# deepinv/deepinv

Hardware: NVIDIA H100
Metric: pnp_pgd_iterations_per_s (higher is better)
Workload: dtype f32 (3 x FP16 split-operand tensor-core GEMMs: 22-bit operands, fp32 accumulate) + f32 operators

## Files before the change

deepinv_b200/csrc/conv_tc32.cu:

```cuda
#include "common.cuh"
#ifndef DINVK_EMUL
#include "tc_ptx.cuh"
#include "tma_tile.cuh"
#include <cuda_fp16.h>
#else
namespace dinvk { namespace tc {
inline void ldg256(const void* p, uint32_t (&r)[8]) { std::memcpy(r, p, 32); }
inline void stg256(void* p, const uint32_t (&r)[8]) { std::memcpy(p, r, 32); }
} }
#endif

#include <algorithm>
#include <cstdlib>
#include <cstring>

namespace dinvk {
namespace t32 {

constexpr int TX = 16, TY = 8;
constexpr int A_TILE = 128 * 128;
constexpr int B_TILE = 128 * 128;
constexpr int STAGE = 2 * A_TILE + B_TILE;
constexpr int STAGES = 4;
constexpr int SMEM = STAGES * STAGE + 1024;
constexpr int THREADS = 2 * 128 + 32;

__device__ __forceinline__ float rna_tf32(float x) {
#ifndef DINVK_EMUL
  uint32_t u;
  asm("cvt.rna.tf32.f32 %0, %1;" : "=r"(u) : "f"(x));
  return __uint_as_float(u);
#else
  return __uint_as_float((__float_as_uint(x) + 0x1000u) & 0xffffe000u);
#endif
}

struct FmtTF32 {
  using elem = float;
  static constexpr int CH = 16, EB = 4, ID = 0;
  static constexpr float CORR = 1.0f;
#ifndef DINVK_EMUL
  static constexpr CUtensorMapDataType TM = CU_TENSOR_MAP_DATA_TYPE_FLOAT32;
#endif
};
struct FmtF16 {
  using elem = __half;
  static constexpr int CH = 32, EB = 2, ID = 1;
  static constexpr float CORR = 4.8828125e-4f;
#ifndef DINVK_EMUL
  static constexpr CUtensorMapDataType TM = CU_TENSOR_MAP_DATA_TYPE_FLOAT16;
#endif
};

#ifndef DINVK_EMUL
template <class F, int N>
__device__ __forceinline__ void mma(float* d, uint32_t a_lo, uint32_t a_hi, uint32_t b_lo, uint32_t b_hi, uint32_t accumulate) {
  if constexpr (F::ID == 0) {
    if constexpr (N == 128) tc::wgmma_tf32_n128(d, a_lo, a_hi, b_lo, b_hi, accumulate);
    else tc::wgmma_tf32_n64(d, a_lo, a_hi, b_lo, b_hi, accumulate);
  } else {
    if constexpr (N == 128) tc::wgmma_f16_n128(d, a_lo, a_hi, b_lo, b_hi, accumulate);
    else tc::wgmma_f16_n64(d, a_lo, a_hi, b_lo, b_hi, accumulate);
  }
}
template <class F>
__device__ __forceinline__ void mma_block(float* acc, uint32_t a, uint32_t a_hi, uint32_t b, uint32_t b_hi, uint32_t fresh) {
  mma<F, 128>(acc, a, a_hi, b, b_hi, fresh);
  mma<F, 128>(acc, a + 2, a_hi, b + 2, b_hi, 1u);
  mma<F, 64>(acc + 32, a + 4, a_hi, b, b_hi, 1u);
  mma<F, 64>(acc + 32, a + 6, a_hi, b + 2, b_hi, 1u);
}
template <class F>
__device__ __forceinline__ void mma_block64(float* acc, uint32_t a, uint32_t a_hi, uint32_t b, uint32_t b_hi, uint32_t fresh) {
  mma<F, 64>(acc, a, a_hi, b, b_hi, fresh);
  mma<F, 64>(acc + 32, a, a_hi, b + 512, b_hi, fresh);
  mma<F, 64>(acc, a + 2, a_hi, b + 2, b_hi, 1u);
  mma<F, 64>(acc + 32, a + 2, a_hi, b + 514, b_hi, 1u);
  mma<F, 64>(acc + 32, a + 4, a_hi, b, b_hi, 1u);
  mma<F, 64>(acc + 32, a + 6, a_hi, b + 2, b_hi, 1u);
}
template <class F>
__device__ __forceinline__ void drain(float* v, const float* acc) {
#pragma unroll
  for (int i = 0; i < 32; ++i) v[i] += acc[i] + acc[32 + i] * F::CORR;
}

__device__ __forceinline__ void release_stage(uint64_t* bar) {
  __syncwarp();
  if ((threadIdx.x & 31) == 0) tc::mbar_arrive(bar);
}

struct Maps {
  CUtensorMap a[4];
  CUtensorMap b;
};

struct Params {
  int B, H, W, Cin, Cout;
  int ntaps, kc_per_tap;
  int dx[9], dy[9], amap[9];
  int mode;
  int tiles_x, tiles_y, n_tiles;
  int relu;
  int win;
  const void* res;
  const void* res2;
  void* out;
  int* flag;
  const float* bias;
  int ngrp;
};

// ... 32 lines not shown
  return bad;
}
template <class F>
__device__ __forceinline__ void add_split_raw(const uint32_t (*raw)[8], float* v) {
  if constexpr (F::ID == 0) {
#pragma unroll
    for (int e = 0; e < 8; ++e) {
      v[e] += __uint_as_float(raw[0][e]) + __uint_as_float(raw[2][e]);
      v[8 + e] += __uint_as_float(raw[1][e]) + __uint_as_float(raw[3][e]);
    }
  } else {
#pragma unroll
    for (int c = 0; c < 2; ++c)
#pragma unroll
      for (int e = 0; e < 8; ++e) {
        const float2 h = __half22float2(*reinterpret_cast<const __half2*>(&raw[c][e]));
        const float2 l = __half22float2(*reinterpret_cast<const __half2*>(&raw[2 + c][e]));
        v[c * 16 + 2 * e] += h.x + l.x * F::CORR;
        v[c * 16 + 2 * e + 1] += h.y + l.y * F::CORR;
      }
  }
}
template <class F>
__device__ __forceinline__ void add_split(const typename F::elem* p, float* v) {
  uint32_t raw[4][8];
  const char* pc = reinterpret_cast<const char*>(p);
#pragma unroll
  for (int k = 0; k < 4; ++k) tc::ldg256(pc + 32 * k, raw[k]);
  add_split_raw<F>(raw, v);
}

#ifndef DINVK_EMUL
template <class F>
__device__ __forceinline__ void add_split_pair(const typename F::elem* p, float& a, float& b) {
  if constexpr (F::ID == 0) {
    const float2 h = __ldg(reinterpret_cast<const float2*>(p)), l = __ldg(reinterpret_cast<const float2*>(p + F::CH));
    a += h.x + l.x;
    b += h.y + l.y;
  } else {
    const float2 h = __half22float2(__ldg(reinterpret_cast<const __half2*>(p)));
    const float2 l = __half22float2(__ldg(reinterpret_cast<const __half2*>(p + F::CH)));
    a += h.x + l.x * F::CORR;
    b += h.y + l.y * F::CORR;
  }
}
template <class F>
__device__ __forceinline__ bool store_split_pair(typename F::elem* p, float a, float b) {
  if constexpr (F::ID == 0) {
    const float ha = rna_tf32(a), hb = rna_tf32(b);
    *reinterpret_cast<float2*>(p) = make_float2(ha, hb);
    *reinterpret_cast<float2*>(p + F::CH) = make_float2(a - ha, b - hb);
    return false;
  } else {
    const __half h0 = __float2half_rn(a), h1 = __float2half_rn(b);
    const __half l0 = __float2half_rn((a - __half2float(h0)) * 2048.0f), l1 = __float2half_rn((b - __half2float(h1)) * 2048.0f);
    *reinterpret_cast<__half2*>(p) = __halves2half2(h0, h1);
    *reinterpret_cast<__half2*>(p + F::CH) = __halves2half2(l0, l1);
    return !(fabsf(a) < 65000.0f) || !(fabsf(b) < 65000.0f);
  }
}

template <class F>
__device__ __forceinline__ void epilogue_split(const Params& P, float* v, int b, const int (&y)[2], const int (&x)[2], int n0) {
  using E = typename F::elem;
  const int q = threadIdx.x & 3;
  const int tap = P.mode == 2 ? n0 / P.Cout : 0;
  const int c0 = n0 - tap * P.Cout;
  bool bad = false;
#pragma unroll
  for (int r = 0; r < 2; ++r) {
    if (!(y[r] < P.H && x[r] < P.W)) continue;
    long long pix;
    if (P.mode == 2) pix = ((long long)b * (2 * P.H) + 2 * y[r] + (tap >> 1)) * (2LL * P.W) + 2 * x[r] + (tap & 1);
    else pix = ((long long)b * P.H + y[r]) * P.W + x[r];
#pragma unroll
    for (int j = 0; j < 8; ++j) {
      const int c = c0 + 8 * j + 2 * q;
      float a = v[4 * j + 2 * r], bb = v[4 * j + 2 * r + 1];
      if (P.bias) { a += __ldg(P.bias + c); bb += __ldg(P.bias + c + 1); }
      if (P.relu) { a = fmaxf(a, 0.f); bb = fmaxf(bb, 0.f); }
      const long long o = pix * P.Cout * 2 + (c / F::CH) * 2 * F::CH + (c % F::CH);
      if (P.res) add_split_pair<F>(static_cast<const E*>(P.res) + o, a, bb);
      if (P.res2) add_split_pair<F>(static_cast<const E*>(P.res2) + o, a, bb);
      bad |= store_split_pair<F>(static_cast<E*>(P.out) + o, a, bb);
    }
  }
  if (bad && P.flag) atomicOr(P.flag, 1);
}

template <class F>
__global__ void __launch_bounds__(THREADS, 1) conv_tc32_kernel(const __grid_constant__ Maps M, const Params P) {
  extern __shared__ uint8_t smem_raw[];
  uint8_t* smem = reinterpret_cast<uint8_t*>((reinterpret_cast<uintptr_t>(smem_raw) + 1023) & ~static_cast<uintptr_t>(1023));
  __shared__ __align__(8) uint64_t full_bar[STAGES];
  __shared__ __align__(8) uint64_t empty_bar[STAGES];

  const int warp = threadIdx.x >> 5, lane = threadIdx.x & 31;
  const int pixel_tiles = P.B * P.tiles_y * P.tiles_x;
  const int total_tiles = pixel_tiles * P.n_tiles;
  const int nk = P.ntaps * P.kc_per_tap;

  if (threadIdx.x == 0) {
    tc::prefetch_tmap(&M.a[0]);
    tc::prefetch_tmap(&M.b);
    for (int s = 0; s < STAGES; ++s) { tc::mbar_init(&full_bar[s], 1); tc::mbar_init(&empty_bar[s], 8); }
    tc::fence_barrier_init();
  }
  __syncthreads();

  if (warp == 8) {
    if (lane == 0) {
      int s = 0; uint32_t ph = 0;
      for (int t = blockIdx.x; t < total_tiles; t += gridDim.x) {
        int pt, nt; tile_index(P, pixel_tiles, t, pt, nt);
        const int b = pt / (P.tiles_y * P.tiles_x), r = pt - b * (P.tiles_y * P.tiles_x);
        const int y0 = (r / P.tiles_x) * TY, x0 = (r % P.tiles_x) * TX;
        for (int kb = 0; kb < nk; ++kb) {
          const int tap = kb / P.kc_per_tap, kc = kb - tap * P.kc_per_tap;
          tc::mbar_wait(&empty_bar[s], ph ^ 1);
          uint8_t* sa = smem + s * STAGE;
          tc::mbar_arrive_expect_tx(&full_bar[s], STAGE);
          tc::tma_load_4d(sa, &M.a[P.amap[tap]], &full_bar[s], (2 * kc) * (2 * F::CH), x0 + P.dx[tap], y0 + P.dy[tap], b);
          tc::tma_load_4d(sa + A_TILE, &M.a[P.amap[tap]], &full_bar[s], (2 * kc + 1) * (2 * F::CH), x0 + P.dx[tap], y0 + P.dy[tap], b);
          tc::tma_load_2d(sa + 2 * A_TILE, &M.b, &full_bar[s], tap * P.Cin + kc * (2 * F::CH), nt * 128);
          if (++s == STAGES) { s = 0; ph ^= 1; }
        }
      }
    }
  } else {
    const int wg = warp >> 2;
    constexpr uint32_t HI = tc::desc_hi_sw128(1024);
    const uint32_t smem_lo = tc::smem_u32(smem) >> 4;
    float acc[64], v[32];
#pragma unroll
    for (int i = 0; i < 64; ++i) acc[i] = 0.f;
    int s = 0; uint32_t ph = 0;
    for (int t = blockIdx.x; t < total_tiles; t += gridDim.x) {
      int pt, nt; tile_index(P, pixel_tiles, t, pt, nt);
      const int b = pt / (P.tiles_y * P.tiles_x), r = pt - b * (P.tiles_y * P.tiles_x);
      const int y0 = (r / P.tiles_x) * TY, x0 = (r % P.tiles_x) * TX;
#pragma unroll
      for (int i = 0; i < 32; ++i) v[i] = 0.f;
      int in_win = 0, pend = -1;
      for (int kb = 0; kb < nk; ++kb) {
        tc::mbar_wait(&full_bar[s], ph);
        const uint32_t a0 = smem_lo + static_cast<uint32_t>(s) * (STAGE >> 4) + static_cast<uint32_t>(wg * (64 * 128 >> 4));
        const uint32_t b0 = smem_lo + static_cast<uint32_t>(s) * (STAGE >> 4) + (2 * A_TILE >> 4);
        tc::wgmma_fence();
#pragma unroll
        for (int jj = 0; jj < 2; ++jj)
          mma_block<F>(acc, a0 + jj * (A_TILE >> 4), HI, b0 + jj * 4, HI, (jj | in_win) != 0 ? 1u : 0u);
        tc::wgmma_commit();
        if (++in_win == P.win || kb == nk - 1) {
          tc::wgmma_wait<0>();
          tc::reg_fence<64>(acc);
          if (pend >= 0) release_stage(&empty_bar[pend]);
          release_stage(&empty_bar[s]);
          pend = -1;
          drain<F>(v, acc);
          in_win = 0;
        } else {
          tc::wgmma_wait<1>();
          if (pend >= 0) release_stage(&empty_bar[pend]);
          pend = s;
        }
        if (++s == STAGES) { s = 0; ph ^= 1; }
      }
      int y[2], x[2];
#pragma unroll
      for (int rr = 0; rr < 2; ++rr) {
        const int m = 64 * wg + 16 * (warp & 3) + (lane >> 2) + 8 * rr;
        y[rr] = y0 + m / TX; x[rr] = x0 + m % TX;
      }
      epilogue_split<F>(P, v, b, y, x, nt * 64);
    }
  }
}

namespace slab {
constexpr int TXP = 16, TYP = 16;
constexpr int SLAB_X = TXP + 8, SLAB_Y = TYP + 2;
constexpr int SLAB_BYTES = SLAB_X * SLAB_Y * 128;
constexpr int A_STAGES = 2, B_STAGES = 6;
constexpr int WT_TILE = 128 * 128;
constexpr int SMEM_BYTES = A_STAGES * SLAB_BYTES + B_STAGES * WT_TILE + 1024;
constexpr int CONSUMER_WARPS = 8;
constexpr int THREADS = 32 * CONSUMER_WARPS + 128;
constexpr int PRODUCER_REGS = 40, CONSUMER_REGS = 232;
static_assert(SLAB_BYTES % 1024 == 0, "slab stages must stay 1024-byte aligned");
static_assert(SMEM_BYTES <= 227 * 1024, "shared memory budget");
}

template <class F>
__global__ void __launch_bounds__(slab::THREADS, 1) conv_tc32_slab_kernel(const __grid_constant__ Maps M, const Params P) {
  using namespace slab;
  extern __shared__ uint8_t smem_raw[];
  uint8_t* smem = reinterpret_cast<uint8_t*>((reinterpret_cast<uintptr_t>(smem_raw) + 1023) & ~static_cast<uintptr_t>(1023));
  uint8_t* smem_b = smem + A_STAGES * SLAB_BYTES;
  __shared__ __align__(8) uint64_t afull[A_STAGES];
  __shared__ __align__(8) uint64_t aempty[A_STAGES];
  __shared__ __align__(8) uint64_t bfull[B_STAGES];
  __shared__ __align__(8) uint64_t bempty[B_STAGES];

  const int warp = threadIdx.x >> 5, lane = threadIdx.x & 31;
  const int pixel_tiles = P.B * P.tiles_y * P.tiles_x;
  const int total_tiles = pixel_tiles * P.n_tiles;
  const int nblk = P.Cin / F::CH;

  if (threadIdx.x == 0) {
    tc::prefetch_tmap(&M.a[0]);
    tc::prefetch_tmap(&M.b);
    for (int s = 0; s < A_STAGES; ++s) { tc::mbar_init(&afull[s], 1); tc::mbar_init(&aempty[s], CONSUMER_WARPS); }
    for (int s = 0; s < B_STAGES; ++s) { tc::mbar_init(&bfull[s], 1); tc::mbar_init(&bempty[s], CONSUMER_WARPS); }
    tc::fence_barrier_init();
  }
  __syncthreads();

  if (warp >= CONSUMER_WARPS) {
    tc::setmaxnreg_dec<PRODUCER_REGS>();
// ... 51 lines not shown
          tc::wgmma_fence();
#pragma unroll
          for (int par = 0; par < 2; ++par) {
            const int tap = 2 * tp + par;
            if (tap < 9) {
              const uint32_t a_t = slab_lo + static_cast<uint32_t>((tap / 3) * SLAB_X + (tap % 3)) * 8;
              mma_block64<F>(acc0, a_t, HI_A, b_lo + par * 4, HI_B, tap == 0 ? fresh : 1u);
              mma_block64<F>(acc1, a_t + BLK1, HI_A, b_lo + par * 4, HI_B, tap == 0 ? fresh : 1u);
            }
          }
          tc::wgmma_commit();
          if (tp == 4) {
            tc::wgmma_wait<0>();
            tc::reg_fence<64>(acc0);
            tc::reg_fence<64>(acc1);
            if (pend_b >= 0) release_stage(&bempty[pend_b]);
            release_stage(&bempty[sb]);
            release_stage(&aempty[sa]);
            pend_b = -1;
            if (last_of_win) {
              drain<F>(v0, acc0);
              drain<F>(v1, acc1);
            }
          } else {
            tc::wgmma_wait<1>();
            if (pend_b >= 0) release_stage(&bempty[pend_b]);
            pend_b = sb;
          }
          if (++sb == B_STAGES) { sb = 0; phb ^= 1; }
        }
        if (++sa == A_STAGES) { sa = 0; pha ^= 1; }
        in_win = last_of_win ? 0 : in_win + 1;
      }
      int y[2], x[2];
#pragma unroll
      for (int rr = 0; rr < 2; ++rr) {
        const int m = 16 * (warp & 3) + (lane >> 2) + 8 * rr;
        y[rr] = y0 + 8 * wg + (m >> 3); x[rr] = x0 + (m & 7);
      }
      epilogue_split<F>(P, v0, b, y, x, nt * 64);
#pragma unroll
      for (int rr = 0; rr < 2; ++rr) x[rr] += 8;
      epilogue_split<F>(P, v1, b, y, x, nt * 64);
    }
  }
}

#endif
struct HeadParams {
  const float* x; const float* w; const float* bias; void* out;
  int B, C, H, W, Cout;
  float fill_scalar; const float* fill_batch; int has_fill; int relu;
  int* flag;
};

template <class F, int CT>
__global__ void __launch_bounds__(256) head_tc32_kernel(const HeadParams P) {
  constexpr int KR = 9 * CT, KP = (KR + 3) & ~3;
#ifndef DINVK_EMUL
  extern __shared__ __align__(16) float sw[];
#else
  float* sw = reinterpret_cast<float*>(::emul::dyn_smem());
#endif
  for (int i = threadIdx.x; i < P.Cout * KP; i += blockDim.x) {
    const int co = i / KP, k = i - co * KP;
    sw[i] = k < KR ? __ldg(P.w + co * KR + k) : 0.f;
  }
  __syncthreads();
  const long long npix = (long long)P.B * P.H * P.W;
  const long long p = (long long)blockIdx.x * blockDim.x + threadIdx.x;
  if (p >= npix) return;
  const long long HW = (long long)P.H * P.W;
  const int b = (int)(p / HW);
  const int rem = (int)(p - (long long)b * HW);
  const int y = rem / P.W, x = rem - y * P.W;
  const float fillv = P.has_fill ? (P.fill_batch ? __ldg(P.fill_batch + b) : P.fill_scalar) : 0.f;
// ... 363 lines not shown
    out[(b * C + c) * HW + hw] = (float)s[0] + (float)s[F::CH] * F::CORR;
  }
}
template <class F>
__global__ void __launch_bounds__(256) nchw_to_split_kernel(const float* __restrict__ in, typename F::elem* __restrict__ out, int C, int H, int W,
                                                            long long n) {
  const long long stride = (long long)gridDim.x * blockDim.x;
  const long long HW = (long long)H * W;
  for (long long i = (long long)blockIdx.x * blockDim.x + threadIdx.x; i < n; i += stride) {
    const long long pix = i / C;
    const int c = (int)(i - pix * C);
    const long long b = pix / HW, hw = pix - b * HW;
    const float v = __ldg(in + (b * C + c) * HW + hw);
    typename F::elem* d = out + pix * C * 2 + (c / F::CH) * 2 * F::CH + (c % F::CH);
    if constexpr (F::ID == 0) {
      const float hi = rna_tf32(v);
      d[0] = hi;
      d[F::CH] = v - hi;
    } else {
      const __half hi = __float2half_rn(v);
      d[0] = hi;
      d[F::CH] = __float2half_rn((v - __half2float(hi)) * 2048.0f);
    }
  }
}

#ifndef DINVK_EMUL
template <class F>
static int map_split(CUtensorMap* m, const void* ptr, int rank, const uint64_t* dims, const uint64_t* strides, const uint32_t* box,
                     const char* what) {
  return encode_tiled(m, F::TM, rank, ptr, dims, strides, box, CU_TENSOR_MAP_SWIZZLE_128B, CU_TENSOR_MAP_L2_PROMOTION_L2_256B, what);
}

static int default_window() {
  static int w = -1;
  if (w < 0) {
    const char* e = getenv("DINVK_TC32_WINDOW");
    w = e ? std::max(1, atoi(e)) : 4;
  }
  return w;
}

template <class F>
static int conv_generic(const void* x, const void* weight, const float* bias, const void* res, const void* res2, void* out, int B, int H,
                        int W, int Cin, int Cout, int kind, int act, int window, int* flag, void* stream) {
  DINVK_CHECK_ARG(x && weight && out, "conv_tc32: null pointer");
  DINVK_CHECK_ARG(B >= 0 && H >= 1 && W >= 1, "conv_tc32: bad shape");
  DINVK_CHECK_ARG(kind >= 0 && kind <= 2, "conv_tc32: kind=%d not in 0..2", kind);
  DINVK_CHECK_ARG(Cin % (2 * F::CH) == 0 && Cin >= 2 * F::CH, "conv_tc32: Cin=%d must be a multiple of %d", Cin, 2 * F::CH);
  DINVK_CHECK_ARG(Cout % 64 == 0 && Cout >= 64, "conv_tc32: Cout=%d must be a multiple of 64", Cout);
  DINVK_CHECK_ARG(kind != 1 || (H % 2 == 0 && W % 2 == 0), "conv_tc32: 2x2 stride-2 needs even H, W");
  DINVK_CHECK_ARG(kind == 0 || (!res && !res2), "conv_tc32: residual inputs are for kind 0 only");
  if (B == 0) return DINVK_OK;
  Maps M;
  Params P{};
  int rc;
  const uint64_t px = (uint64_t)Cin * 2 * F::EB;
  P.B = B; P.Cin = Cin; P.Cout = Cout;
  P.kc_per_tap = Cin / (2 * F::CH);
  P.relu = act; P.res = res; P.res2 = res2; P.out = out; P.bias = bias; P.flag = flag;
  P.win = window > 0 ? window : default_window();
  const uint32_t abox[4] = {2 * F::CH, TX, TY, 1};
  long long K = Cin, rows = 2LL * Cout;
  if (kind == 1) {
    const int Ho = H / 2, Wo = W / 2;
    const uint64_t adims[4] = {(uint64_t)Cin * 2, (uint64_t)Wo, (uint64_t)Ho, (uint64_t)B}, astrides[3] = {2 * px, 2 * px * W, px * W * H};
    for (int t = 0; t < 4; ++t) {
      const char* base = reinterpret_cast<const char*>(x) + ((long long)(t >> 1) * W + (t & 1)) * px;
      if ((rc = map_split<F>(&M.a[t], base, 4, adims, astrides, abox, "tc32 activations"))) return rc;
      P.amap[t] = t;
    }
    K = 4LL * Cin;
    P.H = Ho; P.W = Wo; P.ntaps = 4; P.n_tiles = Cout / 64;
  } else {
    const uint64_t adims[4] = {(uint64_t)Cin * 2, (uint64_t)W, (uint64_t)H, (uint64_t)B}, astrides[3] = {px, px * W, px * W * H};
    if ((rc = map_split<F>(&M.a[0], x, 4, adims, astrides, abox, "tc32 activations"))) return rc;
    M.a[1] = M.a[0]; M.a[2] = M.a[0]; M.a[3] = M.a[0];
    P.H = H; P.W = W;
    if (kind == 0) {
      K = 9LL * Cin;
      P.ntaps = 9; P.n_tiles = Cout / 64;
      for (int t = 0; t < 9; ++t) { P.dx[t] = t % 3 - 1; P.dy[t] = t / 3 - 1; }
    } else {
      rows = 8LL * Cout;
      P.ntaps = 1; P.mode = 2; P.n_tiles = 4 * Cout / 64;
    }
  }
  const uint64_t wdims[2] = {(uint64_t)K, (uint64_t)rows}, wstride = (uint64_t)K * F::EB;
  const uint32_t wbox[2] = {2 * F::CH, 128};
  if ((rc = map_split<F>(&M.b, weight, 2, wdims, &wstride, wbox, "tc32 weights"))) return rc;
  P.tiles_x = ceil_div(P.W, TX); P.tiles_y = ceil_div(P.H, TY);
  P.ngrp = getenv("DINVK_TC32_NT_OUTER") ? 1 : P.n_tiles;
  return launch_persistent(conv_tc32_kernel<F>, THREADS, SMEM, (long long)P.B * P.tiles_y * P.tiles_x * P.n_tiles, stream, M, P);
}

template <class F>
static int conv_slab(const void* x, const void* weight, const float* bias, const void* res, const void* res2, void* out, int B, int H, int W,
                     int Cin, int Cout, int act, int window, int* flag, void* stream) {
  DINVK_CHECK_ARG(x && weight && out, "conv_tc32_slab: null pointer");
  DINVK_CHECK_ARG(B >= 0 && H >= 1 && W >= 1, "conv_tc32_slab: bad shape");
  DINVK_CHECK_ARG(Cin % F::CH == 0 && Cin >= F::CH, "conv_tc32_slab: Cin=%d must be a multiple of %d", Cin, F::CH);
  DINVK_CHECK_ARG(Cout % 64 == 0 && Cout >= 64, "conv_tc32_slab: Cout=%d must be a multiple of 64", Cout);
  if (B == 0) return DINVK_OK;
  Maps M;
  Params P{};
  int rc;
  const uint64_t px = (uint64_t)Cin * 2 * F::EB;
  const uint64_t adims[4] = {(uint64_t)Cin * 2, (uint64_t)W, (uint64_t)H, (uint64_t)B}, astrides[3] = {px, px * W, px * W * H};
  const uint32_t abox[4] = {2 * F::CH, slab::SLAB_X, slab::SLAB_Y, 1};
  if ((rc = map_split<F>(&M.a[0], x, 4, adims, astrides, abox, "tc32 activations"))) return rc;
  M.a[1] = M.a[0]; M.a[2] = M.a[0]; M.a[3] = M.a[0];
  const uint64_t wdims[2] = {10ull * Cin, 2ull * Cout}, wstride = 10ull * Cin * F::EB;
  const uint32_t wbox[2] = {2 * F::CH, 128};
  if ((rc = map_split<F>(&M.b, weight, 2, wdims, &wstride, wbox, "tc32 weights"))) return rc;
  P.B = B; P.H = H; P.W = W; P.Cin = Cin; P.Cout = Cout;
  P.ntaps = 9; P.kc_per_tap = Cin / F::CH; P.n_tiles = Cout / 64;
  for (int t = 0; t < 9; ++t) { P.dx[t] = t % 3 - 1; P.dy[t] = t / 3 - 1; }
  P.relu = act; P.res = res; P.res2 = res2; P.out = out; P.bias = bias; P.flag = flag;
  static const int def_win = getenv("DINVK_TC32_SLAB_WINDOW") ? std::max(1, atoi(getenv("DINVK_TC32_SLAB_WINDOW"))) : 1;
  P.win = window > 0 ? window : def_win;
  P.tiles_x = ceil_div(W, slab::TXP); P.tiles_y = ceil_div(H, slab::TYP);
  {
    static const int env_g = getenv("DINVK_TC32_NT_GROUP") ? atoi(getenv("DINVK_TC32_NT_GROUP")) : 0;
    int g = env_g > 0 ? env_g : (P.n_tiles <= 2 ? P.n_tiles : 1);
    while (g > 1 && P.n_tiles % g) --g;
    P.ngrp = std::max(1, std::min(g, P.n_tiles));
  }
  return launch_persistent(conv_tc32_slab_kernel<F>, slab::THREADS, slab::SMEM_BYTES, (long long)P.B * P.tiles_y * P.tiles_x * P.n_tiles,
                           stream, M, P);
}

#endif
template <class F>
static int conv_head(const float* x_nchw, const float* weight, const float* bias, void* out, int B, int C, int H, int W, int Cout,
                     float fill_scalar, const float* fill_batch, int has_fill, int act, int* flag, void* stream) {
// ... 130 lines not shown
```

deepinv_b200/csrc/tc_ptx.cuh:

```cuda
#pragma once
#include <cstdint>
#include <cuda.h>
#include <cuda_bf16.h>
#include <cuda_runtime.h>

namespace dinvk {
namespace tc {

__device__ __forceinline__ uint32_t smem_u32(const void* p) { return static_cast<uint32_t>(__cvta_generic_to_shared(p)); }

__device__ __forceinline__ bool elect_one() {
  uint32_t pred = 0;
  asm volatile(
      "{\n\t"
      ".reg .pred P;\n\t"
      "elect.sync _|P, 0xffffffff;\n\t"
      "selp.u32 %0, 1, 0, P;\n\t"
      "}\n"
      : "=r"(pred));
  return pred != 0;
}

__device__ __forceinline__ void mbar_init(uint64_t* bar, uint32_t count) {
  asm volatile("mbarrier.init.shared::cta.b64 [%0], %1;" ::"r"(smem_u32(bar)), "r"(count));
// ... 77 lines not shown
        "+f"(d[16]), "+f"(d[17]), "+f"(d[18]), "+f"(d[19]), "+f"(d[20]), "+f"(d[21]), "+f"(d[22]), "+f"(d[23]),
        "+f"(d[24]), "+f"(d[25]), "+f"(d[26]), "+f"(d[27]), "+f"(d[28]), "+f"(d[29]), "+f"(d[30]), "+f"(d[31])
      : "r"(a_lo | (1u << 16)), "r"(a_hi), "r"(b_lo | (1u << 16)), "r"(b_hi), "r"(scale_d)
      : "memory");
}
__device__ __forceinline__ void wgmma_bf16_n128(float* d, uint32_t a_lo, uint32_t a_hi, uint32_t b_lo, uint32_t b_hi, uint32_t scale_d) {
  asm volatile(
      "{\n\t.reg .pred p;\n\t.reg .b64 da, db;\n\t"
      "mov.b64 da, {%64, %65};\n\tmov.b64 db, {%66, %67};\n\tsetp.ne.b32 p, %68, 0;\n\t"
      "wgmma.mma_async.sync.aligned.m64n128k16.f32.bf16.bf16 {%0, %1, %2, %3, %4, %5, %6, %7, %8, %9, %10, %11, %12, %13, %14, %15, %16, %17, %18, %19, %20, %21, %22, %23, %24, %25, %26, %27, %28, %29, %30, %31, %32, %33, %34, %35, %36, %37, %38, %39, %40, %41, %42, %43, %44, %45, %46, %47, %48, %49, %50, %51, %52, %53, %54, %55, %56, %57, %58, %59, %60, %61, %62, %63}, da, db, p, 1, 1, 0, 0;\n\t}\n"
      : "+f"(d[0]), "+f"(d[1]), "+f"(d[2]), "+f"(d[3]), "+f"(d[4]), "+f"(d[5]), "+f"(d[6]), "+f"(d[7]),
        "+f"(d[8]), "+f"(d[9]), "+f"(d[10]), "+f"(d[11]), "+f"(d[12]), "+f"(d[13]), "+f"(d[14]), "+f"(d[15]),
        "+f"(d[16]), "+f"(d[17]), "+f"(d[18]), "+f"(d[19]), "+f"(d[20]), "+f"(d[21]), "+f"(d[22]), "+f"(d[23]),
        "+f"(d[24]), "+f"(d[25]), "+f"(d[26]), "+f"(d[27]), "+f"(d[28]), "+f"(d[29]), "+f"(d[30]), "+f"(d[31]),
        "+f"(d[32]), "+f"(d[33]), "+f"(d[34]), "+f"(d[35]), "+f"(d[36]), "+f"(d[37]), "+f"(d[38]), "+f"(d[39]),
        "+f"(d[40]), "+f"(d[41]), "+f"(d[42]), "+f"(d[43]), "+f"(d[44]), "+f"(d[45]), "+f"(d[46]), "+f"(d[47]),
        "+f"(d[48]), "+f"(d[49]), "+f"(d[50]), "+f"(d[51]), "+f"(d[52]), "+f"(d[53]), "+f"(d[54]), "+f"(d[55]),
        "+f"(d[56]), "+f"(d[57]), "+f"(d[58]), "+f"(d[59]), "+f"(d[60]), "+f"(d[61]), "+f"(d[62]), "+f"(d[63])
      : "r"(a_lo | (1u << 16)), "r"(a_hi), "r"(b_lo | (1u << 16)), "r"(b_hi), "r"(scale_d)
      : "memory");
}
__device__ __forceinline__ void wgmma_f16_n64(float* d, uint32_t a_lo, uint32_t a_hi, uint32_t b_lo, uint32_t b_hi, uint32_t scale_d) {
  asm volatile(
      "{\n\t.reg .pred p;\n\t.reg .b64 da, db;\n\t"
      "mov.b64 da, {%32, %33};\n\tmov.b64 db, {%34, %35};\n\tsetp.ne.b32 p, %36, 0;\n\t"
      "wgmma.mma_async.sync.aligned.m64n64k16.f32.f16.f16 {%0, %1, %2, %3, %4, %5, %6, %7, %8, %9, %10, %11, %12, %13, %14, %15, %16, %17, %18, %19, %20, %21, %22, %23, %24, %25, %26, %27, %28, %29, %30, %31}, da, db, p, 1, 1, 0, 0;\n\t}\n"
      : "+f"(d[0]), "+f"(d[1]), "+f"(d[2]), "+f"(d[3]), "+f"(d[4]), "+f"(d[5]), "+f"(d[6]), "+f"(d[7]),
        "+f"(d[8]), "+f"(d[9]), "+f"(d[10]), "+f"(d[11]), "+f"(d[12]), "+f"(d[13]), "+f"(d[14]), "+f"(d[15]),
        "+f"(d[16]), "+f"(d[17]), "+f"(d[18]), "+f"(d[19]), "+f"(d[20]), "+f"(d[21]), "+f"(d[22]), "+f"(d[23]),
        "+f"(d[24]), "+f"(d[25]), "+f"(d[26]), "+f"(d[27]), "+f"(d[28]), "+f"(d[29]), "+f"(d[30]), "+f"(d[31])
      : "r"(a_lo | (1u << 16)), "r"(a_hi), "r"(b_lo | (1u << 16)), "r"(b_hi), "r"(scale_d)
      : "memory");
}
__device__ __forceinline__ void wgmma_f16_n128(float* d, uint32_t a_lo, uint32_t a_hi, uint32_t b_lo, uint32_t b_hi, uint32_t scale_d) {
  asm volatile(
      "{\n\t.reg .pred p;\n\t.reg .b64 da, db;\n\t"
      "mov.b64 da, {%64, %65};\n\tmov.b64 db, {%66, %67};\n\tsetp.ne.b32 p, %68, 0;\n\t"
      "wgmma.mma_async.sync.aligned.m64n128k16.f32.f16.f16 {%0, %1, %2, %3, %4, %5, %6, %7, %8, %9, %10, %11, %12, %13, %14, %15, %16, %17, %18, %19, %20, %21, %22, %23, %24, %25, %26, %27, %28, %29, %30, %31, %32, %33, %34, %35, %36, %37, %38, %39, %40, %41, %42, %43, %44, %45, %46, %47, %48, %49, %50, %51, %52, %53, %54, %55, %56, %57, %58, %59, %60, %61, %62, %63}, da, db, p, 1, 1, 0, 0;\n\t}\n"
      : "+f"(d[0]), "+f"(d[1]), "+f"(d[2]), "+f"(d[3]), "+f"(d[4]), "+f"(d[5]), "+f"(d[6]), "+f"(d[7]),
        "+f"(d[8]), "+f"(d[9]), "+f"(d[10]), "+f"(d[11]), "+f"(d[12]), "+f"(d[13]), "+f"(d[14]), "+f"(d[15]),
        "+f"(d[16]), "+f"(d[17]), "+f"(d[18]), "+f"(d[19]), "+f"(d[20]), "+f"(d[21]), "+f"(d[22]), "+f"(d[23]),
        "+f"(d[24]), "+f"(d[25]), "+f"(d[26]), "+f"(d[27]), "+f"(d[28]), "+f"(d[29]), "+f"(d[30]), "+f"(d[31]),
        "+f"(d[32]), "+f"(d[33]), "+f"(d[34]), "+f"(d[35]), "+f"(d[36]), "+f"(d[37]), "+f"(d[38]), "+f"(d[39]),
        "+f"(d[40]), "+f"(d[41]), "+f"(d[42]), "+f"(d[43]), "+f"(d[44]), "+f"(d[45]), "+f"(d[46]), "+f"(d[47]),
        "+f"(d[48]), "+f"(d[49]), "+f"(d[50]), "+f"(d[51]), "+f"(d[52]), "+f"(d[53]), "+f"(d[54]), "+f"(d[55]),
        "+f"(d[56]), "+f"(d[57]), "+f"(d[58]), "+f"(d[59]), "+f"(d[60]), "+f"(d[61]), "+f"(d[62]), "+f"(d[63])
      : "r"(a_lo | (1u << 16)), "r"(a_hi), "r"(b_lo | (1u << 16)), "r"(b_hi), "r"(scale_d)
      : "memory");
}
__device__ __forceinline__ void wgmma_tf32_n64(float* d, uint32_t a_lo, uint32_t a_hi, uint32_t b_lo, uint32_t b_hi, uint32_t scale_d) {
  asm volatile(
      "{\n\t.reg .pred p;\n\t.reg .b64 da, db;\n\t"
      "mov.b64 da, {%32, %33};\n\tmov.b64 db, {%34, %35};\n\tsetp.ne.b32 p, %36, 0;\n\t"
      "wgmma.mma_async.sync.aligned.m64n64k8.f32.tf32.tf32 {%0, %1, %2, %3, %4, %5, %6, %7, %8, %9, %10, %11, %12, %13, %14, %15, %16, %17, %18, %19, %20, %21, %22, %23, %24, %25, %26, %27, %28, %29, %30, %31}, da, db, p, 1, 1;\n\t}\n"
      : "+f"(d[0]), "+f"(d[1]), "+f"(d[2]), "+f"(d[3]), "+f"(d[4]), "+f"(d[5]), "+f"(d[6]), "+f"(d[7]),
        "+f"(d[8]), "+f"(d[9]), "+f"(d[10]), "+f"(d[11]), "+f"(d[12]), "+f"(d[13]), "+f"(d[14]), "+f"(d[15]),
        "+f"(d[16]), "+f"(d[17]), "+f"(d[18]), "+f"(d[19]), "+f"(d[20]), "+f"(d[21]), "+f"(d[22]), "+f"(d[23]),
        "+f"(d[24]), "+f"(d[25]), "+f"(d[26]), "+f"(d[27]), "+f"(d[28]), "+f"(d[29]), "+f"(d[30]), "+f"(d[31])
      : "r"(a_lo | (1u << 16)), "r"(a_hi), "r"(b_lo | (1u << 16)), "r"(b_hi), "r"(scale_d)
      : "memory");
}
__device__ __forceinline__ void wgmma_tf32_n128(float* d, uint32_t a_lo, uint32_t a_hi, uint32_t b_lo, uint32_t b_hi, uint32_t scale_d) {
  asm volatile(
      "{\n\t.reg .pred p;\n\t.reg .b64 da, db;\n\t"
      "mov.b64 da, {%64, %65};\n\tmov.b64 db, {%66, %67};\n\tsetp.ne.b32 p, %68, 0;\n\t"
      "wgmma.mma_async.sync.aligned.m64n128k8.f32.tf32.tf32 {%0, %1, %2, %3, %4, %5, %6, %7, %8, %9, %10, %11, %12, %13, %14, %15, %16, %17, %18, %19, %20, %21, %22, %23, %24, %25, %26, %27, %28, %29, %30, %31, %32, %33, %34, %35, %36, %37, %38, %39, %40, %41, %42, %43, %44, %45, %46, %47, %48, %49, %50, %51, %52, %53, %54, %55, %56, %57, %58, %59, %60, %61, %62, %63}, da, db, p, 1, 1;\n\t}\n"
      : "+f"(d[0]), "+f"(d[1]), "+f"(d[2]), "+f"(d[3]), "+f"(d[4]), "+f"(d[5]), "+f"(d[6]), "+f"(d[7]),
        "+f"(d[8]), "+f"(d[9]), "+f"(d[10]), "+f"(d[11]), "+f"(d[12]), "+f"(d[13]), "+f"(d[14]), "+f"(d[15]),
        "+f"(d[16]), "+f"(d[17]), "+f"(d[18]), "+f"(d[19]), "+f"(d[20]), "+f"(d[21]), "+f"(d[22]), "+f"(d[23]),
        "+f"(d[24]), "+f"(d[25]), "+f"(d[26]), "+f"(d[27]), "+f"(d[28]), "+f"(d[29]), "+f"(d[30]), "+f"(d[31]),
        "+f"(d[32]), "+f"(d[33]), "+f"(d[34]), "+f"(d[35]), "+f"(d[36]), "+f"(d[37]), "+f"(d[38]), "+f"(d[39]),
        "+f"(d[40]), "+f"(d[41]), "+f"(d[42]), "+f"(d[43]), "+f"(d[44]), "+f"(d[45]), "+f"(d[46]), "+f"(d[47]),
        "+f"(d[48]), "+f"(d[49]), "+f"(d[50]), "+f"(d[51]), "+f"(d[52]), "+f"(d[53]), "+f"(d[54]), "+f"(d[55]),
        "+f"(d[56]), "+f"(d[57]), "+f"(d[58]), "+f"(d[59]), "+f"(d[60]), "+f"(d[61]), "+f"(d[62]), "+f"(d[63])
      : "r"(a_lo | (1u << 16)), "r"(a_hi), "r"(b_lo | (1u << 16)), "r"(b_hi), "r"(scale_d)
      : "memory");
}

__device__ __forceinline__ void ldg256(const void* p, uint32_t (&r)[8]) {
  const uint4 a = __ldg(reinterpret_cast<const uint4*>(p)), b = __ldg(reinterpret_cast<const uint4*>(p) + 1);
  r[0] = a.x; r[1] = a.y; r[2] = a.z; r[3] = a.w; r[4] = b.x; r[5] = b.y; r[6] = b.z; r[7] = b.w;
}
__device__ __forceinline__ void stg256(void* p, const uint32_t (&r)[8]) {
  reinterpret_cast<uint4*>(p)[0] = make_uint4(r[0], r[1], r[2], r[3]);
  reinterpret_cast<uint4*>(p)[1] = make_uint4(r[4], r[5], r[6], r[7]);
}

}
}
```

Before: 7.112.

## Stage epilogue through shared memory for 16-byte vectorized split stores

Both conv kernels now write their accumulator fragments into a per-warp swizzled shared-memory buffer before the epilogue. Each lane then reads back contiguous channel runs, so bias, residual loads and the hi/lo split stores become 16-byte vector accesses instead of scattered 8-byte pairs. The tiled kernel also drops its N=128 wgmma shapes in favour of N=64 blocks, and it now waits on every k-block and releases the stage right away instead of keeping one group in flight. That removes MMA/TMA overlap and may cost speed, in exchange for fewer live registers and simpler code. A host check now requires 16-byte alignment of bias, res, res2 and out, and shared memory grows by the staging buffers.

Result: faster. 7.336, median of 6 (+3.2%).

```diff
diff --git a/deepinv_b200/csrc/conv_tc32.cu b/deepinv_b200/csrc/conv_tc32.cu
--- a/deepinv_b200/csrc/conv_tc32.cu
+++ b/deepinv_b200/csrc/conv_tc32.cu
@@ -22,7 +22,8 @@
 constexpr int B_TILE = 128 * 128;
 constexpr int STAGE = 2 * A_TILE + B_TILE;
 constexpr int STAGES = 4;
-constexpr int SMEM = STAGES * STAGE + 1024;
+constexpr int STG_WARP = 16 * 32;
+constexpr int SMEM = STAGES * STAGE + 8 * STG_WARP * 4 + 1024;
 constexpr int THREADS = 2 * 128 + 32;
 
 __device__ __forceinline__ float rna_tf32(float x) {
@@ -53,31 +54,19 @@
 };
 
 #ifndef DINVK_EMUL
-template <class F, int N>
+template <class F>
 __device__ __forceinline__ void mma(float* d, uint32_t a_lo, uint32_t a_hi, uint32_t b_lo, uint32_t b_hi, uint32_t accumulate) {
-  if constexpr (F::ID == 0) {
-    if constexpr (N == 128) tc::wgmma_tf32_n128(d, a_lo, a_hi, b_lo, b_hi, accumulate);
-    else tc::wgmma_tf32_n64(d, a_lo, a_hi, b_lo, b_hi, accumulate);
-  } else {
-    if constexpr (N == 128) tc::wgmma_f16_n128(d, a_lo, a_hi, b_lo, b_hi, accumulate);
-    else tc::wgmma_f16_n64(d, a_lo, a_hi, b_lo, b_hi, accumulate);
-  }
-}
-template <class F>
-__device__ __forceinline__ void mma_block(float* acc, uint32_t a, uint32_t a_hi, uint32_t b, uint32_t b_hi, uint32_t fresh) {
-  mma<F, 128>(acc, a, a_hi, b, b_hi, fresh);
-  mma<F, 128>(acc, a + 2, a_hi, b + 2, b_hi, 1u);
-  mma<F, 64>(acc + 32, a + 4, a_hi, b, b_hi, 1u);
-  mma<F, 64>(acc + 32, a + 6, a_hi, b + 2, b_hi, 1u);
+  if constexpr (F::ID == 0) tc::wgmma_tf32_n64(d, a_lo, a_hi, b_lo, b_hi, accumulate);
+  else tc::wgmma_f16_n64(d, a_lo, a_hi, b_lo, b_hi, accumulate);
 }
 template <class F>
 __device__ __forceinline__ void mma_block64(float* acc, uint32_t a, uint32_t a_hi, uint32_t b, uint32_t b_hi, uint32_t fresh) {
-  mma<F, 64>(acc, a, a_hi, b, b_hi, fresh);
-  mma<F, 64>(acc + 32, a, a_hi, b + 512, b_hi, fresh);
-  mma<F, 64>(acc, a + 2, a_hi, b + 2, b_hi, 1u);
-  mma<F, 64>(acc + 32, a + 2, a_hi, b + 514, b_hi, 1u);
-  mma<F, 64>(acc + 32, a + 4, a_hi, b, b_hi, 1u);
-  mma<F, 64>(acc + 32, a + 6, a_hi, b + 2, b_hi, 1u);
+  mma<F>(acc, a, a_hi, b, b_hi, fresh);
+  mma<F>(acc + 32, a, a_hi, b + 512, b_hi, fresh);
+  mma<F>(acc, a + 2, a_hi, b + 2, b_hi, 1u);
+  mma<F>(acc + 32, a + 2, a_hi, b + 514, b_hi, 1u);
+  mma<F>(acc + 32, a + 4, a_hi, b, b_hi, 1u);
+  mma<F>(acc + 32, a + 6, a_hi, b + 2, b_hi, 1u);
 }
 template <class F>
 __device__ __forceinline__ void drain(float* v, const float* acc) {
@@ -176,57 +165,113 @@
 
 #ifndef DINVK_EMUL
 template <class F>
-__device__ __forceinline__ void add_split_pair(const typename F::elem* p, float& a, float& b) {
+__device__ __forceinline__ void add_split16(const uint4& h, const uint4& l, float (&a)[16 / F::EB]) {
   if constexpr (F::ID == 0) {
-    const float2 h = __ldg(reinterpret_cast<const float2*>(p)), l = __ldg(reinterpret_cast<const float2*>(p + F::CH));
-    a += h.x + l.x;
-    b += h.y + l.y;
+    const float* hf = reinterpret_cast<const float*>(&h);
+    const float* lf = reinterpret_cast<const float*>(&l);
+#pragma unroll
+    for (int i = 0; i < 4; ++i) a[i] += hf[i] + lf[i];
   } else {
-    const float2 h = __half22float2(__ldg(reinterpret_cast<const __half2*>(p)));
-    const float2 l = __half22float2(__ldg(reinterpret_cast<const __half2*>(p + F::CH)));
-    a += h.x + l.x * F::CORR;
-    b += h.y + l.y * F::CORR;
-  }
-}
-template <class F>
-__device__ __forceinline__ bool store_split_pair(typename F::elem* p, float a, float b) {
-  if constexpr (F::ID == 0) {
-    const float ha = rna_tf32(a), hb = rna_tf32(b);
-    *reinterpret_cast<float2*>(p) = make_float2(ha, hb);
-    *reinterpret_cast<float2*>(p + F::CH) = make_float2(a - ha, b - hb);
-    return false;
-  } else {
-    const __half h0 = __float2half_rn(a), h1 = __float2half_rn(b);
-    const __half l0 = __float2half_rn((a - __half2float(h0)) * 2048.0f), l1 = __float2half_rn((b - __half2float(h1)) * 2048.0f);
-    *reinterpret_cast<__half2*>(p) = __halves2half2(h0, h1);
-    *reinterpret_cast<__half2*>(p + F::CH) = __halves2half2(l0, l1);
-    return !(fabsf(a) < 65000.0f) || !(fabsf(b) < 65000.0f);
-  }
-}
-
-template <class F>
-__device__ __forceinline__ void epilogue_split(const Params& P, float* v, int b, const int (&y)[2], const int (&x)[2], int n0) {
+    const __half2* h2 = reinterpret_cast<const __half2*>(&h);
+    const __half2* l2 = reinterpret_cast<const __half2*>(&l);
+#pragma unroll
+    for (int i = 0; i < 4; ++i) {
+      const float2 hv = __half22float2(h2[i]), lv = __half22float2(l2[i]);
+      a[2 * i] += hv.x + lv.x * F::CORR;
+      a[2 * i + 1] += hv.y + lv.y * F::CORR;
+    }
+  }
+}
+template <class F>
+__device__ __forceinline__ bool store_split16(typename F::elem* p, const float (&a)[16 / F::EB]) {
+  uint32_t h[4], l[4];
+  bool bad = false;
+#pragma unroll
+  for (int i = 0; i < 4; ++i) {
+    if constexpr (F::ID == 0) {
+      const float hi = rna_tf32(a[i]);
+      h[i] = __float_as_uint(hi);
+      l[i] = __float_as_uint(a[i] - hi);
+    } else {
+      const float a0 = a[2 * i], a1 = a[2 * i + 1];
+      const __half h0 = __float2half_rn(a0), h1 = __float2half_rn(a1);
+      const __half l0 = __float2half_rn((a0 - __half2float(h0)) * 2048.0f), l1 = __float2half_rn((a1 - __half2float(h1)) * 2048.0f);
+      h[i] = (uint32_t)__half_as_ushort(h0) | ((uint32_t)__half_as_ushort(h1) << 16);
+      l[i] = (uint32_t)__half_as_ushort(l0) | ((uint32_t)__half_as_ushort(l1) << 16);
+      bad |= !(fabsf(a0) < 65000.0f) || !(fabsf(a1) < 65000.0f);
+    }
+  }
+  *reinterpret_cast<uint4*>(p) = make_uint4(h[0], h[1], h[2], h[3]);
+  *reinterpret_cast<uint4*>(p + F::CH) = make_uint4(l[0], l[1], l[2], l[3]);
+  return bad;
+}
+
+__device__ __forceinline__ int stg_off(int r, int k) { return 32 * r + 4 * (k ^ ((2 * r & 6) | ((r >> 2) & 1))); }
+
+template <class F, class PixelOf>
+__device__ __forceinline__ void epilogue(const Params& P, const float* v, float* stg, PixelOf pixel_of, int c0) {
   using E = typename F::elem;
-  const int q = threadIdx.x & 3;
-  const int tap = P.mode == 2 ? n0 / P.Cout : 0;
-  const int c0 = n0 - tap * P.Cout;
+  constexpr int K = 16 / F::EB, NP = 16 / K;
+  const int lane = threadIdx.x & 31, q = lane & 3;
+  const int rl = F::ID == 0 ? lane >> 3 : lane & 7;
+  const int cl = F::ID == 0 ? lane & 7 : lane >> 3;
+  long long pix[NP];
+#pragma unroll
+  for (int p = 0; p < NP; ++p) pix[p] = pixel_of(rl + K * p);
   bool bad = false;
 #pragma unroll
-  for (int r = 0; r < 2; ++r) {
-    if (!(y[r] < P.H && x[r] < P.W)) continue;
-    long long pix;
-    if (P.mode == 2) pix = ((long long)b * (2 * P.H) + 2 * y[r] + (tap >> 1)) * (2LL * P.W) + 2 * x[r] + (tap & 1);
-    else pix = ((long long)b * P.H + y[r]) * P.W + x[r];
-#pragma unroll
-    for (int j = 0; j < 8; ++j) {
-      const int c = c0 + 8 * j + 2 * q;
-      float a = v[4 * j + 2 * r], bb = v[4 * j + 2 * r + 1];
-      if (P.bias) { a += __ldg(P.bias + c); bb += __ldg(P.bias + c + 1); }
-      if (P.relu) { a = fmaxf(a, 0.f); bb = fmaxf(bb, 0.f); }
-      const long long o = pix * P.Cout * 2 + (c / F::CH) * 2 * F::CH + (c % F::CH);
-      if (P.res) add_split_pair<F>(static_cast<const E*>(P.res) + o, a, bb);
-      if (P.res2) add_split_pair<F>(static_cast<const E*>(P.res2) + o, a, bb);
-      bad |= store_split_pair<F>(static_cast<E*>(P.out) + o, a, bb);
+  for (int half = 0; half < 2; ++half) {
+    const int c = c0 + 32 * half + K * cl;
+    const long long oc = (c / F::CH) * 2 * F::CH + (c % F::CH);
+    float4 bv[K / 4];
+    uint4 r1[NP][2], r2[NP][2];
+#pragma unroll
+    for (int k = 0; k < K / 4; ++k) bv[k] = P.bias ? __ldg(reinterpret_cast<const float4*>(P.bias + c) + k) : make_float4(0.f, 0.f, 0.f, 0.f);
+#pragma unroll
+    for (int p = 0; p < NP; ++p) {
+      r1[p][0] = r1[p][1] = r2[p][0] = r2[p][1] = make_uint4(0u, 0u, 0u, 0u);
+      if (pix[p] < 0) continue;
+      const long long o = pix[p] * P.Cout * 2 + oc;
+      if (P.res) {
+        r1[p][0] = __ldg(reinterpret_cast<const uint4*>(static_cast<const E*>(P.res) + o));
+        r1[p][1] = __ldg(reinterpret_cast<const uint4*>(static_cast<const E*>(P.res) + o + F::CH));
+      }
+      if (P.res2) {
+        r2[p][0] = __ldg(reinterpret_cast<const uint4*>(static_cast<const E*>(P.res2) + o));
+        r2[p][1] = __ldg(reinterpret_cast<const uint4*>(static_cast<const E*>(P.res2) + o + F::CH));
+      }
+    }
+    __syncwarp();
+#pragma unroll
+    for (int j = 0; j < 4; ++j)
+#pragma unroll
+      for (int h = 0; h < 2; ++h) {
+        const int i = 4 * (4 * half + j) + 2 * h;
+        *reinterpret_cast<float2*>(stg + stg_off((lane >> 2) + 8 * h, 2 * j + (q >> 1)) + 2 * (q & 1)) = make_float2(v[i], v[i + 1]);
+      }
+    __syncwarp();
+#pragma unroll
+    for (int p = 0; p < NP; ++p) {
+      if (pix[p] < 0) continue;
+      float a[K];
+#pragma unroll
+      for (int k = 0; k < K / 4; ++k) {
+        const float4 s = *reinterpret_cast<const float4*>(stg + stg_off(rl + K * p, K / 4 * cl + k));
+        a[4 * k] = s.x; a[4 * k + 1] = s.y; a[4 * k + 2] = s.z; a[4 * k + 3] = s.w;
+      }
+      if (P.bias) {
+#pragma unroll
+        for (int k = 0; k < K / 4; ++k) {
+          a[4 * k] += bv[k].x; a[4 * k + 1] += bv[k].y; a[4 * k + 2] += bv[k].z; a[4 * k + 3] += bv[k].w;
+        }
+      }
+      if (P.relu) {
+#pragma unroll
+        for (int e = 0; e < K; ++e) a[e] = fmaxf(a[e], 0.f);
+      }
+      if (P.res) add_split16<F>(r1[p][0], r1[p][1], a);
+      if (P.res2) add_split16<F>(r2[p][0], r2[p][1], a);
+      bad |= store_split16<F>(static_cast<E*>(P.out) + pix[p] * P.Cout * 2 + oc, a);
     }
   }
   if (bad && P.flag) atomicOr(P.flag, 1);
@@ -275,17 +320,17 @@
     const int wg = warp >> 2;
     constexpr uint32_t HI = tc::desc_hi_sw128(1024);
     const uint32_t smem_lo = tc::smem_u32(smem) >> 4;
-    float acc[64], v[32];
-#pragma unroll
-    for (int i = 0; i < 64; ++i) acc[i] = 0.f;
     int s = 0; uint32_t ph = 0;
     for (int t = blockIdx.x; t < total_tiles; t += gridDim.x) {
       int pt, nt; tile_index(P, pixel_tiles, t, pt, nt);
       const int b = pt / (P.tiles_y * P.tiles_x), r = pt - b * (P.tiles_y * P.tiles_x);
       const int y0 = (r / P.tiles_x) * TY, x0 = (r % P.tiles_x) * TX;
+      float acc[64], v[32];
+#pragma unroll
+      for (int i = 0; i < 64; ++i) acc[i] = 0.f;
 #pragma unroll
       for (int i = 0; i < 32; ++i) v[i] = 0.f;
-      int in_win = 0, pend = -1;
+      int in_win = 0;
       for (int kb = 0; kb < nk; ++kb) {
         tc::mbar_wait(&full_bar[s], ph);
         const uint32_t a0 = smem_lo + static_cast<uint32_t>(s) * (STAGE >> 4) + static_cast<uint32_t>(wg * (64 * 128 >> 4));
@@ -293,30 +338,26 @@
         tc::wgmma_fence();
 #pragma unroll
         for (int jj = 0; jj < 2; ++jj)
-          mma_block<F>(acc, a0 + jj * (A_TILE >> 4), HI, b0 + jj * 4, HI, (jj | in_win) != 0 ? 1u : 0u);
+          mma_block64<F>(acc, a0 + jj * (A_TILE >> 4), HI, b0 + jj * 4, HI, (jj | in_win) != 0 ? 1u : 0u);
         tc::wgmma_commit();
+        tc::wgmma_wait<0>();
+        tc::reg_fence<64>(acc);
+        release_stage(&empty_bar[s]);
         if (++in_win == P.win || kb == nk - 1) {
-          tc::wgmma_wait<0>();
-          tc::reg_fence<64>(acc);
-          if (pend >= 0) release_stage(&empty_bar[pend]);
-          release_stage(&empty_bar[s]);
-          pend = -1;
           drain<F>(v, acc);
           in_win = 0;
-        } else {
-          tc::wgmma_wait<1>();
-          if (pend >= 0) release_stage(&empty_bar[pend]);
-          pend = s;
         }
         if (++s == STAGES) { s = 0; ph ^= 1; }
       }
-      int y[2], x[2];
-#pragma unroll
-      for (int rr = 0; rr < 2; ++rr) {
-        const int m = 64 * wg + 16 * (warp & 3) + (lane >> 2) + 8 * rr;
-        y[rr] = y0 + m / TX; x[rr] = x0 + m % TX;
-      }
-      epilogue_split<F>(P, v, b, y, x, nt * 64);
+      const int tap = P.mode == 2 ? nt * 64 / P.Cout : 0;
+      const auto pixel_of = [&](int m) -> long long {
+        const int mm = 64 * wg + 16 * (warp & 3) + m;
+        const int y = y0 + mm / TX, x = x0 + mm % TX;
+        if (!(y < P.H && x < P.W)) return -1;
+        if (P.mode == 2) return ((long long)b * (2 * P.H) + 2 * y + (tap >> 1)) * (2LL * P.W) + 2 * x + (tap & 1);
+        return ((long long)b * P.H + y) * P.W + x;
+      };
+      epilogue<F>(P, v, reinterpret_cast<float*>(smem + STAGES * STAGE) + warp * STG_WARP, pixel_of, nt * 64 - tap * P.Cout);
     }
   }
 }
@@ -327,8 +368,8 @@
 constexpr int SLAB_BYTES = SLAB_X * SLAB_Y * 128;
 constexpr int A_STAGES = 2, B_STAGES = 6;
 constexpr int WT_TILE = 128 * 128;
-constexpr int SMEM_BYTES = A_STAGES * SLAB_BYTES + B_STAGES * WT_TILE + 1024;
 constexpr int CONSUMER_WARPS = 8;
+constexpr int SMEM_BYTES = A_STAGES * SLAB_BYTES + B_STAGES * WT_TILE + CONSUMER_WARPS * STG_WARP * 4 + 1024;
 constexpr int THREADS = 32 * CONSUMER_WARPS + 128;
 constexpr int PRODUCER_REGS = 40, CONSUMER_REGS = 232;
 static_assert(SLAB_BYTES % 1024 == 0, "slab stages must stay 1024-byte aligned");
@@ -446,16 +487,16 @@
         if (++sa == A_STAGES) { sa = 0; pha ^= 1; }
         in_win = last_of_win ? 0 : in_win + 1;
       }
-      int y[2], x[2];
-#pragma unroll
-      for (int rr = 0; rr < 2; ++rr) {
-        const int m = 16 * (warp & 3) + (lane >> 2) + 8 * rr;
-        y[rr] = y0 + 8 * wg + (m >> 3); x[rr] = x0 + (m & 7);
-      }
-      epilogue_split<F>(P, v0, b, y, x, nt * 64);
-#pragma unroll
-      for (int rr = 0; rr < 2; ++rr) x[rr] += 8;
-      epilogue_split<F>(P, v1, b, y, x, nt * 64);
+      float* stg = reinterpret_cast<float*>(smem_b + B_STAGES * WT_TILE) + warp * STG_WARP;
+#pragma unroll
+      for (int blk = 0; blk < 2; ++blk) {
+        const auto pixel_of = [&](int m) -> long long {
+          const int mm = 16 * (warp & 3) + m;
+          const int y = y0 + 8 * wg + (mm >> 3), x = x0 + 8 * blk + (mm & 7);
+          return y < P.H && x < P.W ? ((long long)b * P.H + y) * P.W + x : -1;
+        };
+        epilogue<F>(P, blk ? v1 : v0, stg, pixel_of, nt * 64);
+      }
     }
   }
 }
@@ -885,6 +926,12 @@
   return encode_tiled(m, F::TM, rank, ptr, dims, strides, box, CU_TENSOR_MAP_SWIZZLE_128B, CU_TENSOR_MAP_L2_PROMOTION_L2_256B, what);
 }
 
+static bool epilogue_aligned(const float* bias, const void* res, const void* res2, const void* out) {
+  const uintptr_t any = reinterpret_cast<uintptr_t>(bias) | reinterpret_cast<uintptr_t>(res) | reinterpret_cast<uintptr_t>(res2) |
+                        reinterpret_cast<uintptr_t>(out);
+  return (any & 15) == 0;
+}
+
 static int default_window() {
   static int w = -1;
   if (w < 0) {
@@ -904,6 +951,7 @@
   DINVK_CHECK_ARG(Cout % 64 == 0 && Cout >= 64, "conv_tc32: Cout=%d must be a multiple of 64", Cout);
   DINVK_CHECK_ARG(kind != 1 || (H % 2 == 0 && W % 2 == 0), "conv_tc32: 2x2 stride-2 needs even H, W");
   DINVK_CHECK_ARG(kind == 0 || (!res && !res2), "conv_tc32: residual inputs are for kind 0 only");
+  DINVK_CHECK_ARG(epilogue_aligned(bias, res, res2, out), "conv_tc32: bias, res, res2 and out must be 16-byte aligned");
   if (B == 0) return DINVK_OK;
   Maps M;
   Params P{};
@@ -954,6 +1002,7 @@
   DINVK_CHECK_ARG(B >= 0 && H >= 1 && W >= 1, "conv_tc32_slab: bad shape");
   DINVK_CHECK_ARG(Cin % F::CH == 0 && Cin >= F::CH, "conv_tc32_slab: Cin=%d must be a multiple of %d", Cin, F::CH);
   DINVK_CHECK_ARG(Cout % 64 == 0 && Cout >= 64, "conv_tc32_slab: Cout=%d must be a multiple of 64", Cout);
+  DINVK_CHECK_ARG(epilogue_aligned(bias, res, res2, out), "conv_tc32_slab: bias, res, res2 and out must be 16-byte aligned");
   if (B == 0) return DINVK_OK;
   Maps M;
   Params P{};
diff --git a/deepinv_b200/csrc/tc_ptx.cuh b/deepinv_b200/csrc/tc_ptx.cuh
--- a/deepinv_b200/csrc/tc_ptx.cuh
+++ b/deepinv_b200/csrc/tc_ptx.cuh
@@ -133,22 +133,6 @@
       : "r"(a_lo | (1u << 16)), "r"(a_hi), "r"(b_lo | (1u << 16)), "r"(b_hi), "r"(scale_d)
       : "memory");
 }
-__device__ __forceinline__ void wgmma_f16_n128(float* d, uint32_t a_lo, uint32_t a_hi, uint32_t b_lo, uint32_t b_hi, uint32_t scale_d) {
-  asm volatile(
-      "{\n\t.reg .pred p;\n\t.reg .b64 da, db;\n\t"
-      "mov.b64 da, {%64, %65};\n\tmov.b64 db, {%66, %67};\n\tsetp.ne.b32 p, %68, 0;\n\t"
-      "wgmma.mma_async.sync.aligned.m64n128k16.f32.f16.f16 {%0, %1, %2, %3, %4, %5, %6, %7, %8, %9, %10, %11, %12, %13, %14, %15, %16, %17, %18, %19, %20, %21, %22, %23, %24, %25, %26, %27, %28, %29, %30, %31, %32, %33, %34, %35, %36, %37, %38, %39, %40, %41, %42, %43, %44, %45, %46, %47, %48, %49, %50, %51, %52, %53, %54, %55, %56, %57, %58, %59, %60, %61, %62, %63}, da, db, p, 1, 1, 0, 0;\n\t}\n"
-      : "+f"(d[0]), "+f"(d[1]), "+f"(d[2]), "+f"(d[3]), "+f"(d[4]), "+f"(d[5]), "+f"(d[6]), "+f"(d[7]),
-        "+f"(d[8]), "+f"(d[9]), "+f"(d[10]), "+f"(d[11]), "+f"(d[12]), "+f"(d[13]), "+f"(d[14]), "+f"(d[15]),
-        "+f"(d[16]), "+f"(d[17]), "+f"(d[18]), "+f"(d[19]), "+f"(d[20]), "+f"(d[21]), "+f"(d[22]), "+f"(d[23]),
-        "+f"(d[24]), "+f"(d[25]), "+f"(d[26]), "+f"(d[27]), "+f"(d[28]), "+f"(d[29]), "+f"(d[30]), "+f"(d[31]),
-        "+f"(d[32]), "+f"(d[33]), "+f"(d[34]), "+f"(d[35]), "+f"(d[36]), "+f"(d[37]), "+f"(d[38]), "+f"(d[39]),
-        "+f"(d[40]), "+f"(d[41]), "+f"(d[42]), "+f"(d[43]), "+f"(d[44]), "+f"(d[45]), "+f"(d[46]), "+f"(d[47]),
-        "+f"(d[48]), "+f"(d[49]), "+f"(d[50]), "+f"(d[51]), "+f"(d[52]), "+f"(d[53]), "+f"(d[54]), "+f"(d[55]),
-        "+f"(d[56]), "+f"(d[57]), "+f"(d[58]), "+f"(d[59]), "+f"(d[60]), "+f"(d[61]), "+f"(d[62]), "+f"(d[63])
-      : "r"(a_lo | (1u << 16)), "r"(a_hi), "r"(b_lo | (1u << 16)), "r"(b_hi), "r"(scale_d)
-      : "memory");
-}
 __device__ __forceinline__ void wgmma_tf32_n64(float* d, uint32_t a_lo, uint32_t a_hi, uint32_t b_lo, uint32_t b_hi, uint32_t scale_d) {
   asm volatile(
       "{\n\t.reg .pred p;\n\t.reg .b64 da, db;\n\t"
@@ -158,22 +142,6 @@
         "+f"(d[8]), "+f"(d[9]), "+f"(d[10]), "+f"(d[11]), "+f"(d[12]), "+f"(d[13]), "+f"(d[14]), "+f"(d[15]),
         "+f"(d[16]), "+f"(d[17]), "+f"(d[18]), "+f"(d[19]), "+f"(d[20]), "+f"(d[21]), "+f"(d[22]), "+f"(d[23]),
         "+f"(d[24]), "+f"(d[25]), "+f"(d[26]), "+f"(d[27]), "+f"(d[28]), "+f"(d[29]), "+f"(d[30]), "+f"(d[31])
-      : "r"(a_lo | (1u << 16)), "r"(a_hi), "r"(b_lo | (1u << 16)), "r"(b_hi), "r"(scale_d)
-      : "memory");
-}
-__device__ __forceinline__ void wgmma_tf32_n128(float* d, uint32_t a_lo, uint32_t a_hi, uint32_t b_lo, uint32_t b_hi, uint32_t scale_d) {
-  asm volatile(
-      "{\n\t.reg .pred p;\n\t.reg .b64 da, db;\n\t"
-      "mov.b64 da, {%64, %65};\n\tmov.b64 db, {%66, %67};\n\tsetp.ne.b32 p, %68, 0;\n\t"
-      "wgmma.mma_async.sync.aligned.m64n128k8.f32.tf32.tf32 {%0, %1, %2, %3, %4, %5, %6, %7, %8, %9, %10, %11, %12, %13, %14, %15, %16, %17, %18, %19, %20, %21, %22, %23, %24, %25, %26, %27, %28, %29, %30, %31, %32, %33, %34, %35, %36, %37, %38, %39, %40, %41, %42, %43, %44, %45, %46, %47, %48, %49, %50, %51, %52, %53, %54, %55, %56, %57, %58, %59, %60, %61, %62, %63}, da, db, p, 1, 1;\n\t}\n"
-      : "+f"(d[0]), "+f"(d[1]), "+f"(d[2]), "+f"(d[3]), "+f"(d[4]), "+f"(d[5]), "+f"(d[6]), "+f"(d[7]),
-        "+f"(d[8]), "+f"(d[9]), "+f"(d[10]), "+f"(d[11]), "+f"(d[12]), "+f"(d[13]), "+f"(d[14]), "+f"(d[15]),
-        "+f"(d[16]), "+f"(d[17]), "+f"(d[18]), "+f"(d[19]), "+f"(d[20]), "+f"(d[21]), "+f"(d[22]), "+f"(d[23]),
-        "+f"(d[24]), "+f"(d[25]), "+f"(d[26]), "+f"(d[27]), "+f"(d[28]), "+f"(d[29]), "+f"(d[30]), "+f"(d[31]),
-        "+f"(d[32]), "+f"(d[33]), "+f"(d[34]), "+f"(d[35]), "+f"(d[36]), "+f"(d[37]), "+f"(d[38]), "+f"(d[39]),
-        "+f"(d[40]), "+f"(d[41]), "+f"(d[42]), "+f"(d[43]), "+f"(d[44]), "+f"(d[45]), "+f"(d[46]), "+f"(d[47]),
-        "+f"(d[48]), "+f"(d[49]), "+f"(d[50]), "+f"(d[51]), "+f"(d[52]), "+f"(d[53]), "+f"(d[54]), "+f"(d[55]),
-        "+f"(d[56]), "+f"(d[57]), "+f"(d[58]), "+f"(d[59]), "+f"(d[60]), "+f"(d[61]), "+f"(d[62]), "+f"(d[63])
       : "r"(a_lo | (1u << 16)), "r"(a_hi), "r"(b_lo | (1u << 16)), "r"(b_hi), "r"(scale_d)
       : "memory");
 }
```
